# tyiannak/pyAudioAnalysis

Hardware: NVIDIA H100
Metric: audio frames/sec short-term feature_extraction @16kHz 50/25ms (higher is better)
Workload: dtype f32

## Files before the change

pyaudioanalysis_b200/csrc/b200aa.cu:

```cuda
#include <cuda_runtime.h>
#include <nvtx3/nvToolsExt.h>

#include <algorithm>
#include <atomic>
#include <cmath>
#include <cstdio>
#include <cstring>
#include <map>
#include <memory>
#include <mutex>
#include <string>
#include <vector>

#include "../../include/b200aa.h"
#include "beat.cuh"
#include "common.cuh"
#include "generic_kernel.cuh"
#include "fast_kernel.cuh"
#include "pair_kernel.cuh"
#include "pcm.cuh"
#include "solo_kernel.cuh"
#include "tables.inl"

using namespace b200aa;

static thread_local std::string g_cuda_err;
static std::atomic<int64_t> g_launches{0};

static int cuda_fail(cudaError_t e, const char *what)
{
    g_cuda_err = std::string(what) + ": " + cudaGetErrorString(e);
    return B200AA_ERR_CUDA;
}
#define CK(call)                                                     \
    do {                                                             \
        cudaError_t e_ = (call);                                     \
        if (e_ != cudaSuccess) return cuda_fail(e_, #call);          \
    } while (0)
#define CK_LAUNCH(name)                                              \
    do {                                                             \
        g_launches.fetch_add(1, std::memory_order_relaxed);          \
        cudaError_t e_ = cudaGetLastError();                         \
        if (e_ != cudaSuccess) return cuda_fail(e_, name);           \
    } while (0)

struct NvtxRange {
    explicit NvtxRange(const char *name) { nvtxRangePushA(name); }
    ~NvtxRange() { nvtxRangePop(); }
};

extern "C" int b200aa_abi_version(void) { return B200AA_ABI_VERSION; }
extern "C" int64_t b200aa_launch_count(void) { return g_launches.load(); }
extern "C" const char *b200aa_last_cuda_error(void) { return g_cuda_err.c_str(); }

extern "C" const char *b200aa_status_string(int s)
{
    switch (s) {
    case B200AA_OK: return "ok";
    case B200AA_ERR_INVALID: return "invalid argument";
    case B200AA_ERR_TOO_SHORT: return "need at least one array to concatenate";
    case B200AA_ERR_CHROMA: return "chroma: semitone index >= num_fft (window too short for this sampling rate)";
    case B200AA_ERR_MEL_RANGE: return "mel filterbank: filter edge beyond num_fft";
    case B200AA_ERR_CUDA: return "CUDA error";
    case B200AA_ERR_UNSUPPORTED: return "window too large for the on-chip transform";
    case B200AA_ERR_NO_DEVICE: return "no sm_90 CUDA device";
    default: return "unknown status";
    }
}

extern "C" int b200aa_device_ok(void)
{
    int dev = 0;
    if (cudaGetDevice(&dev) != cudaSuccess) { cudaGetLastError(); return B200AA_ERR_NO_DEVICE; }
    cudaDeviceProp pr;
    if (cudaGetDeviceProperties(&pr, dev) != cudaSuccess) { cudaGetLastError(); return B200AA_ERR_NO_DEVICE; }
    return (pr.major == 9 && pr.minor == 0) ? B200AA_OK : B200AA_ERR_NO_DEVICE;
}

extern "C" int b200aa_host_table(int fs, int window, int which, double *h_out)
{
    if (!h_out || window < 2 || fs <= 0) return B200AA_ERR_INVALID;
    const int K = window / 2;
    std::vector<double> t;
    int rc = B200AA_OK;
    if (which == 0) rc = b200aa_host::build_mel(fs, K, t);
    else if (which == 1) rc = b200aa_host::build_chroma(fs, K, t);
    else if (which == 2) b200aa_host::build_dct(t);
    else return B200AA_ERR_INVALID;
    if (rc != B200AA_OK) return rc;
    std::memcpy(h_out, t.data(), t.size() * sizeof(double));
    return B200AA_OK;
}

extern "C" int64_t b200aa_num_frames(int64_t n, int w, int s)
{
    return (w < 1 || s < 1) ? 0 : b200aa_host::num_frames(n, w, s);
}
extern "C" int64_t b200aa_spectrogram_rows(int64_t n, int w, int s)
{
    return (w < 1 || s < 1) ? 0 : rows::spectrogram(n, w, s).R;
}
extern "C" int64_t b200aa_chromagram_rows(int64_t n, int w, int s)
{
    return (w < 1 || s < 1) ? 0 : rows::chromagram(n, w, s).R;
}
__host__ __device__ inline int64_t frames_of(int64_t n, int w, int s) { return n < w ? 0 : (n - w) / s + 1; }
__host__ __device__ inline int64_t windows_of(int64_t n_frames, int stepr)
{
    return (stepr < 1 || n_frames <= 0) ? 0 : (n_frames + stepr - 1) / stepr;
}

extern "C" int64_t b200aa_mid_windows(int64_t n_frames, int stepr) { return windows_of(n_frames, stepr); }

struct Transform {
    int n = 0, Nc = 0, packed = 0;
    std::vector<int> radix;
    float2 *d_tw = nullptr, *d_tw_post = nullptr;
    ~Transform()
    {
        if (d_tw) cudaFree(d_tw);
        if (d_tw_post) cudaFree(d_tw_post);
    }
};

struct b200aa_plan {
    int fs = 0, window = 0, step = 0, K = 0;
    int device = 0, sm_count = 0;
    int force_generic = 0;
    int fast_kind = 0;
    int tables_status = B200AA_OK;
    BlobLayout bl{};
    int *d_blob = nullptr;
    std::vector<int> h_blob;
    std::mutex mu;
    std::map<int, std::unique_ptr<Transform>> transforms;
    std::mutex host_mu;
    void *ws[4] = {nullptr, nullptr, nullptr, nullptr};
    size_t ws_cap[4] = {0, 0, 0, 0};
    FastTables fast{};
    PairTables pair{};
    SoloTables solo{};
    int prefer = -1;
    static constexpr unsigned kSlots = 64;
    static constexpr size_t kSlotBytes = 64 * 1024;
    unsigned char *d_counters = nullptr;
    cudaEvent_t slot_event[kSlots] = {};
    bool slot_used[kSlots] = {};
    unsigned next_slot = 0;
    std::mutex slot_mu;
    static constexpr int kPipe = 3;
    cudaStream_t pipe_stream[kPipe] = {nullptr, nullptr, nullptr};
    void *pipe_ws[kPipe][3] = {};
    size_t pipe_cap[kPipe][3] = {};
    ~b200aa_plan()
    {
        if (d_blob) cudaFree(d_blob);
        for (void *w : ws) if (w) cudaFree(w);
        for (int k = 0; k < kPipe; ++k) {
            if (pipe_stream[k]) cudaStreamDestroy(pipe_stream[k]);
            for (void *w : pipe_ws[k]) if (w) cudaFree(w);
        }
        fast.release();
        pair.release();
        solo.release();
        if (d_counters) cudaFree(d_counters);
        for (cudaEvent_t e : slot_event) if (e) cudaEventDestroy(e);
    }
};

static int make_transform(int n, std::unique_ptr<Transform> &out)
{
    std::unique_ptr<Transform> t(new Transform);
    t->n = n;
    t->packed = (n % 2 == 0) ? 1 : 0;
    t->Nc = t->packed ? n / 2 : n;
    t->radix = b200aa_host::radix_list(t->Nc);
    if (t->Nc == 1) t->radix.clear();
    if ((int)t->radix.size() > kMaxRadix) return B200AA_ERR_UNSUPPORTED;
    std::vector<float2> tw(t->Nc), tp(t->Nc);
    for (int j = 0; j < t->Nc; ++j) {
        const double a = -2.0 * b200aa_host::kPi * double(j) / double(t->Nc);
        tw[j] = make_float2(float(std::cos(a)), float(std::sin(a)));
        const double b = -2.0 * b200aa_host::kPi * double(j) / double(n);
        tp[j] = make_float2(float(std::cos(b)), float(std::sin(b)));
    }
    CK(cudaMalloc(&t->d_tw, sizeof(float2) * t->Nc));
    CK(cudaMalloc(&t->d_tw_post, sizeof(float2) * t->Nc));
    CK(cudaMemcpy(t->d_tw, tw.data(), sizeof(float2) * t->Nc, cudaMemcpyHostToDevice));
    CK(cudaMemcpy(t->d_tw_post, tp.data(), sizeof(float2) * t->Nc, cudaMemcpyHostToDevice));
    out = std::move(t);
    return B200AA_OK;
}

static int get_transform(b200aa_plan *pl, int n, Transform **out)
{
    std::lock_guard<std::mutex> g(pl->mu);
    auto it = pl->transforms.find(n);
    if (it == pl->transforms.end()) {
        std::unique_ptr<Transform> t;
        int rc = make_transform(n, t);
        if (rc != B200AA_OK) return rc;
        it = pl->transforms.emplace(n, std::move(t)).first;
    }
    *out = it->second.get();
    return B200AA_OK;
}

extern "C" int b200aa_plan_create(b200aa_plan **out, int fs, int window, int step)
{
    if (!out || fs <= 0 || window < 2 || step < 1) return B200AA_ERR_INVALID;
    int rc = b200aa_device_ok();
    if (rc != B200AA_OK) return rc;
    std::unique_ptr<b200aa_plan> pl(new b200aa_plan);
    pl->fs = fs; pl->window = window; pl->step = step; pl->K = window / 2;
    CK(cudaGetDevice(&pl->device));
    CK(cudaDeviceGetAttribute(&pl->sm_count, cudaDevAttrMultiProcessorCount, pl->device));
    pl->tables_status = b200aa_host::build_blob(fs, pl->K, pl->h_blob, pl->bl);
    CK(cudaMalloc(&pl->d_blob, sizeof(int) * pl->h_blob.size()));
    CK(cudaMemcpy(pl->d_blob, pl->h_blob.data(), sizeof(int) * pl->h_blob.size(), cudaMemcpyHostToDevice));
    Transform *t = nullptr;
    rc = get_transform(pl.get(), window, &t);
    if (rc != B200AA_OK) return rc;
    rc = fast_plan_init(fs, window, step, pl->h_blob, pl->bl, &pl->fast, &pl->fast_kind);
    if (rc != B200AA_OK) return rc;
    int sl_ = 0, sr_ = 0;
    if ((pair_r_for_window(window) || solo_shape_for_window(window, &sl_, &sr_)) && pl->tables_status == B200AA_OK) {
        std::vector<double> mel, chr, dct;
        b200aa_host::build_mel(fs, pl->K, mel);
        b200aa_host::build_chroma(fs, pl->K, chr);
        b200aa_host::build_dct(dct);
        std::vector<int> pblob;
        PairBlobLayout pbl{};
        build_pair_blob(mel, chr, dct, pl->K, pblob, pbl);
        rc = pair_plan_init(window, pblob, pbl, &pl->pair);
        if (rc != B200AA_OK) return cuda_fail(cudaGetLastError(), "pair_plan_init");
        rc = solo_plan_init(window, pblob, pbl, &pl->solo);
        if (rc != B200AA_OK) return cuda_fail(cudaGetLastError(), "solo_plan_init");
    }
    CK(cudaMalloc(&pl->d_counters, b200aa_plan::kSlots * b200aa_plan::kSlotBytes));
    *out = pl.release();
    return B200AA_OK;
}

extern "C" void b200aa_plan_destroy(b200aa_plan *plan) { delete plan; }
static int slot_acquire(b200aa_plan *pl, cudaStream_t st, unsigned *slot, unsigned int **ctr)
{
    std::lock_guard<std::mutex> g(pl->slot_mu);
    const unsigned s = pl->next_slot++ % b200aa_plan::kSlots;
    if (!pl->slot_event[s]) CK(cudaEventCreateWithFlags(&pl->slot_event[s], cudaEventDisableTiming));
    if (pl->slot_used[s]) CK(cudaStreamWaitEvent(st, pl->slot_event[s], 0));
    *slot = s;
    *ctr = reinterpret_cast<unsigned int *>(pl->d_counters + size_t(s) * b200aa_plan::kSlotBytes);
    return B200AA_OK;
}
static int slot_done(b200aa_plan *pl, cudaStream_t st, unsigned slot)
{
    std::lock_guard<std::mutex> g(pl->slot_mu);
    CK(cudaEventRecord(pl->slot_event[slot], st));
    pl->slot_used[slot] = true;
    return B200AA_OK;
}

static bool use_pair(const b200aa_plan *pl) { return pl->pair.R && !pl->force_generic && (pl->prefer < 0 || pl->prefer == 2); }
static bool use_solo(const b200aa_plan *pl) { return pl->solo.L && !pl->force_generic && (pl->prefer < 0 || pl->prefer == 3); }
static bool use_fast(const b200aa_plan *pl) { return pl->fast_kind && !pl->force_generic && (pl->prefer < 0 || pl->prefer == 1); }
extern "C" int b200aa_plan_kernel_kind(const b200aa_plan *plan)
{
    if (!plan) return 0;
    return use_pair(plan) ? 2 : (use_solo(plan) ? 3 : (use_fast(plan) ? 1 : 0));
}
extern "C" int b200aa_plan_prefer_kernel(b200aa_plan *plan, int kind)
{
    if (!plan || kind < -1 || kind > 3) return B200AA_ERR_INVALID;
    plan->prefer = kind;
    return B200AA_OK;
}
static float *g_pair_dump = nullptr;
extern "C" int b200aa_debug_set_dump(float *d_rows)
{
    g_pair_dump = d_rows;
    return B200AA_OK;
}
extern "C" int b200aa_plan_force_generic(b200aa_plan *plan, int on)
{
    if (!plan) return 0;
    int prev = plan->force_generic;
    plan->force_generic = on ? 1 : 0;
    return prev;
}

extern "C" int b200aa_plan_trim(b200aa_plan *plan)
{
    if (!plan) return B200AA_ERR_INVALID;
    std::lock_guard<std::mutex> g(plan->host_mu);
    for (int i = 0; i < 4; ++i) {
        if (plan->ws[i]) cudaFree(plan->ws[i]);
        plan->ws[i] = nullptr; plan->ws_cap[i] = 0;
    }
    for (int k = 0; k < b200aa_plan::kPipe; ++k)
        for (int j = 0; j < 3; ++j) {
            if (plan->pipe_ws[k][j]) cudaFree(plan->pipe_ws[k][j]);
            plan->pipe_ws[k][j] = nullptr; plan->pipe_cap[k][j] = 0;
        }
    return B200AA_OK;
}

static int plan_device_check(const b200aa_plan *pl)
{
    int dev = -1;
    CK(cudaGetDevice(&dev));
    return dev == pl->device ? B200AA_OK : B200AA_ERR_INVALID;
}

__device__ __forceinline__ int float_key(float f)
{
    int b = __float_as_int(f);
    return b >= 0 ? b : b ^ 0x7fffffff;
}
__device__ __forceinline__ float key_float(int k) { return __int_as_float(k >= 0 ? k : k ^ 0x7fffffff); }

__global__ void stats_init_kernel(b200aa_clip_norm *nm, int64_t n)
{
    int64_t i = blockIdx.x * int64_t(blockDim.x) + threadIdx.x;
    if (i >= n) return;
    unsigned long long *acc = reinterpret_cast<unsigned long long *>(&nm[i].rsv[1]);
    *acc = 0ull;
    reinterpret_cast<int *>(&nm[i].lo)[0] = 0x7fffffff;
    reinterpret_cast<int *>(&nm[i].hi)[0] = int(0x80000000u);
}

template <int DTYPE>
__global__ void __launch_bounds__(256) stats_accum_kernel(const void *sig, int64_t n_samples, int64_t clip_stride,
                                                           const int64_t *len, b200aa_clip_norm *nm, int chunks)
{
    const int64_t b = blockIdx.y;
    const int64_t L = len ? len[b] : n_samples;
    const int64_t per = (L + chunks - 1) / chunks;
    const int64_t s0 = blockIdx.x * per, s1 = min(L, s0 + per);
    long long isum = 0;
    double dsum = 0.0;
    int kmin = 0x7fffffff, kmax = int(0x80000000u);
    if (DTYPE == B200AA_DTYPE_I16) {
        const short *x = reinterpret_cast<const short *>(sig) + b * clip_stride;
        int mn = 32767, mx = -32768;
        int64_t i = s0 + threadIdx.x;
        const bool al = ((reinterpret_cast<uintptr_t>(x + s0) & 15) == 0);
        if (al) {
            const int4 *v = reinterpret_cast<const int4 *>(x + s0);
            const int64_t nv = (s1 - s0) / 8;
            int64_t j = threadIdx.x;
            for (; j + 3 * int64_t(blockDim.x) < nv; j += 4 * int64_t(blockDim.x)) {
                int4 q[4];
#pragma unroll
                for (int t = 0; t < 4; ++t) q[t] = __ldg(v + j + t * int64_t(blockDim.x));
                int acc = 0;
#pragma unroll
                for (int t = 0; t < 4; ++t) {
                    const int w4[4] = {q[t].x, q[t].y, q[t].z, q[t].w};
#pragma unroll
                    for (int u = 0; u < 4; ++u) {
                        const int a0 = (short)(w4[u] & 0xffff), a1 = w4[u] >> 16;
                        acc += a0 + a1;
                        mn = min(mn, min(a0, a1));
                        mx = max(mx, max(a0, a1));
                    }
                }
                isum += acc;
            }
            for (; j < nv; j += blockDim.x) {
                int acc = 0;
                const int4 q = __ldg(v + j);
                const int w4[4] = {q.x, q.y, q.z, q.w};
#pragma unroll
                for (int u = 0; u < 4; ++u) {
                    const int a0 = (short)(w4[u] & 0xffff), a1 = w4[u] >> 16;
                    acc += a0 + a1;
                    mn = min(mn, min(a0, a1));
                    mx = max(mx, max(a0, a1));
                }
                isum += acc;
            }
            i = s0 + nv * 8 + threadIdx.x;
        }
        for (; i < s1; i += blockDim.x) {
            const int a0 = x[i];
            isum += a0;
            mn = min(mn, a0);
            mx = max(mx, a0);
        }
        kmin = mn; kmax = mx;
    } else {
        const float *x = reinterpret_cast<const float *>(sig) + b * clip_stride;
        for (int64_t i = s0 + threadIdx.x; i < s1; i += blockDim.x) {
            const float v = x[i];
            dsum += double(v);
            const int k = float_key(v);
            kmin = min(kmin, k);
            kmax = max(kmax, k);
        }
    }
    __shared__ long long s_i[8];
    __shared__ double s_d[8];
    __shared__ int s_mn[8], s_mx[8];
    const int lane = threadIdx.x & 31, warp = threadIdx.x >> 5;
#pragma unroll
    for (int o = 16; o > 0; o >>= 1) {
        isum += __shfl_xor_sync(0xffffffffu, isum, o);
        dsum += __shfl_xor_sync(0xffffffffu, dsum, o);
        kmin = min(kmin, __shfl_xor_sync(0xffffffffu, kmin, o));
        kmax = max(kmax, __shfl_xor_sync(0xffffffffu, kmax, o));
    }
    if (lane == 0) { s_i[warp] = isum; s_d[warp] = dsum; s_mn[warp] = kmin; s_mx[warp] = kmax; }
    __syncthreads();
    if (threadIdx.x == 0 && s1 > s0) {
        for (int w = 1; w < 8; ++w) { isum += s_i[w]; dsum += s_d[w]; kmin = min(kmin, s_mn[w]); kmax = max(kmax, s_mx[w]); }
        if (DTYPE == B200AA_DTYPE_I16)
            atomicAdd(reinterpret_cast<unsigned long long *>(&nm[b].rsv[1]), (unsigned long long)isum);
        else
            atomicAdd(reinterpret_cast<double *>(&nm[b].rsv[1]), dsum);
        atomicMin(reinterpret_cast<int *>(&nm[b].lo), kmin);
        atomicMax(reinterpret_cast<int *>(&nm[b].hi), kmax);
    }
}

template <int DTYPE>
__global__ void stats_finish_kernel(b200aa_clip_norm *nm, int64_t n, int64_t n_samples, const int64_t *len)
{
    int64_t i = blockIdx.x * int64_t(blockDim.x) + threadIdx.x;
    if (i >= n) return;
    const int64_t L = len ? len[i] : n_samples;
    b200aa_clip_norm r = nm[i];
    double mean, mn, mx;
    if (DTYPE == B200AA_DTYPE_I16) {
        const long long s = *reinterpret_cast<const long long *>(&nm[i].rsv[1]);
        mean = L > 0 ? double(s) / double(L) : 0.0;
        mn = double(*reinterpret_cast<const int *>(&r.lo));
        mx = double(*reinterpret_cast<const int *>(&r.hi));
    } else {
        const double s = *reinterpret_cast<const double *>(&nm[i].rsv[1]);
        mean = L > 0 ? s / double(L) : 0.0;
        mn = double(key_float(*reinterpret_cast<const int *>(&r.lo)));
        mx = double(key_float(*reinterpret_cast<const int *>(&r.hi)));
    }
    if (L <= 0) { mn = mx = 0.0; }
    const double maxdev = fmax(mx - mean, mean - mn);
    const double a = 1.0 / (maxdev + 32768.0 * 1e-10);
    double m, lo, hi;
    if (DTYPE == B200AA_DTYPE_I16) {
        m = nearbyint(mean);
        lo = floor(mean);
        hi = ceil(mean);
    } else {
        const float mf = float(mean);
        m = double(mf);
        if (double(mf) > mean) { hi = mf; lo = nextafterf(mf, -INFINITY); }
        else if (double(mf) < mean) { lo = mf; hi = nextafterf(mf, INFINITY); }
        else { lo = hi = mf; }
    }
    b200aa_clip_norm o;
    o.a = float(a);
    o.bp = float(a * (m - mean));
    o.m = float(m);
    o.lo = float(lo - m);
    o.hi = float(hi - m);
    o.rsv[0] = o.rsv[1] = o.rsv[2] = 0.f;
    nm[i] = o;
}

extern "C" int b200aa_clip_stats(const void *d_sig, int dtype, int64_t n_clips, int64_t n_samples,
                                 int64_t clip_stride, const int64_t *d_len, b200aa_clip_norm *d_norm, void *stream)
{
    NvtxRange nvtx_("b200aa_clip_stats");
    if (!d_sig || !d_norm || n_clips < 0 || n_samples < 0 || (dtype != 0 && dtype != 1)) return B200AA_ERR_INVALID;
    if (n_clips == 0) return B200AA_OK;
    cudaStream_t st = static_cast<cudaStream_t>(stream);
    int dev = 0, sms = 0;
    CK(cudaGetDevice(&dev));
    CK(cudaDeviceGetAttribute(&sms, cudaDevAttrMultiProcessorCount, dev));
    const int tb = 256;
    stats_init_kernel<<<(unsigned)((n_clips + tb - 1) / tb), tb, 0, st>>>(d_norm, n_clips);
    CK_LAUNCH("stats_init_kernel");
    int64_t want = (int64_t(sms) * 8 + n_clips - 1) / n_clips;
    const int64_t bytes = n_samples * (dtype == 0 ? 2 : 4);
    int64_t cap = (bytes + 32767) / 32768;
    int chunks = (int)std::max<int64_t>(1, std::min<int64_t>(want, cap));
    for (int64_t b0 = 0; b0 < n_clips; b0 += 32768) {
        const int64_t nb = std::min<int64_t>(32768, n_clips - b0);
        dim3 grid(chunks, (unsigned)nb);
        const size_t es = dtype == 0 ? 2 : 4;
        const void *sig = reinterpret_cast<const char *>(d_sig) + size_t(b0) * clip_stride * es;
        const int64_t *ln = d_len ? d_len + b0 : nullptr;
        if (dtype == 0) stats_accum_kernel<0><<<grid, 256, 0, st>>>(sig, n_samples, clip_stride, ln, d_norm + b0, chunks);
        else stats_accum_kernel<1><<<grid, 256, 0, st>>>(sig, n_samples, clip_stride, ln, d_norm + b0, chunks);
        CK_LAUNCH("stats_accum_kernel");
    }
    if (dtype == 0) stats_finish_kernel<0><<<(unsigned)((n_clips + tb - 1) / tb), tb, 0, st>>>(d_norm, n_clips, n_samples, d_len);
    else stats_finish_kernel<1><<<(unsigned)((n_clips + tb - 1) / tb), tb, 0, st>>>(d_norm, n_clips, n_samples, d_len);
    CK_LAUNCH("stats_finish_kernel");
    return B200AA_OK;
}

template <bool RAGGED>
__global__ void __launch_bounds__(256) mid_pool_kernel(const float *st, int64_t n_clips, int F, int64_t T,
                                                        int64_t t_stride, const int64_t *frames, int ratio, int stepr,
                                                        int64_t M, float *mid)
{
    const int lane = threadIdx.x & 31;
    const int64_t wid = (blockIdx.x * int64_t(blockDim.x) + threadIdx.x) >> 5;
    const int64_t total = n_clips * F * M;
    if (wid >= total) return;
    const int64_t j = wid % M, bf = wid / M;
    const int64_t b = bf / F;
    const int f = int(bf - b * F);
    if (RAGGED) {
        T = min(max(frames[b], int64_t(0)), t_stride);
        if (j >= windows_of(T, stepr)) return;
    }
    const int64_t c0 = j * stepr;
    int64_t c1 = min(T, c0 + ratio);
    if (c1 < 0) c1 = max(c1 + T, int64_t(0));
    const float *row = st + (size_t(b) * F + f) * t_stride;
    const int n = int(max(c1 - c0, int64_t(0)));
    double s = 0.0;
    for (int64_t c = c0 + lane; c < c1; c += 32) s += double(row[c]);
#pragma unroll
    for (int o = 16; o > 0; o >>= 1) s += __shfl_xor_sync(0xffffffffu, s, o);
    const double mean = s / double(n);
    double v = 0.0;
    for (int64_t c = c0 + lane; c < c1; c += 32) { const double d = double(row[c]) - mean; v += d * d; }
#pragma unroll
    for (int o = 16; o > 0; o >>= 1) v += __shfl_xor_sync(0xffffffffu, v, o);
    if (lane == 0) {
        float mu = float(mean), sd = float(sqrt(v / double(n)));
        if (isnan(mu)) mu = 0.f;
        if (isnan(sd)) sd = 0.f;
        if (isinf(mu)) mu = mu > 0 ? 3.4028234664e38f : -3.4028234664e38f;
        if (isinf(sd)) sd = 3.4028234664e38f;
        mid[(size_t(b) * 2 * F + f) * M + j] = mu;
        mid[(size_t(b) * 2 * F + F + f) * M + j] = sd;
    }
}

static int mid_pool_launch(const float *d_st, int64_t n_clips, int n_feats, int64_t T, int64_t t_stride, const int64_t *d_frames,
                           int ratio, int step_ratio, float *d_mid, void *stream)
{
    const int64_t M = windows_of(T, step_ratio);
    const int64_t warps = n_clips * n_feats * M;
    if (warps == 0) return B200AA_OK;
    const int64_t blocks = (warps * 32 + 255) / 256;
    auto kernel = d_frames ? mid_pool_kernel<true> : mid_pool_kernel<false>;
    kernel<<<(unsigned)blocks, 256, 0, static_cast<cudaStream_t>(stream)>>>(d_st, n_clips, n_feats, T, t_stride, d_frames,
                                                                             ratio, step_ratio, M, d_mid);
    CK_LAUNCH("mid_pool_kernel");
    return B200AA_OK;
}

extern "C" int b200aa_mid_pool(const float *d_st, int64_t n_clips, int n_feats, int64_t n_frames, int64_t t_stride,
                               int ratio, int step_ratio, float *d_mid, void *stream)
{
    NvtxRange nvtx_("b200aa_mid_pool");
    if (!d_st || !d_mid || n_clips < 0 || n_feats < 1 || n_frames < 1 || step_ratio < 1 || t_stride < n_frames)
        return B200AA_ERR_INVALID;
    return mid_pool_launch(d_st, n_clips, n_feats, n_frames, t_stride, nullptr, ratio, step_ratio, d_mid, stream);
}

extern "C" int b200aa_mid_pool_ragged(const float *d_st, int64_t n_clips, int n_feats, int64_t t_stride,
                                      const int64_t *d_frames, int ratio, int step_ratio, float *d_mid, void *stream)
{
    NvtxRange nvtx_("b200aa_mid_pool_ragged");
    if (!d_st || !d_frames || !d_mid || n_clips < 0 || n_feats < 1 || step_ratio < 1 || t_stride < 0)
        return B200AA_ERR_INVALID;
    return mid_pool_launch(d_st, n_clips, n_feats, t_stride, t_stride, d_frames, ratio, step_ratio, d_mid, stream);
}

__global__ void __launch_bounds__(256) long_term_mean_kernel(const float *mid, int64_t rows_total, int n_rows, int64_t M,
                                                             const int64_t *windows, float *out)
{
    const int lane = threadIdx.x & 31;
    const int64_t wid = (blockIdx.x * int64_t(blockDim.x) + threadIdx.x) >> 5;
    if (wid >= rows_total) return;
    const int64_t Mb = windows ? min(max(windows[wid / n_rows], int64_t(0)), M) : M;
    const float *row = mid + size_t(wid) * M;
    double s = 0.0;
    for (int64_t c = lane; c < Mb; c += 32) s += double(row[c]);
#pragma unroll
    for (int o = 16; o > 0; o >>= 1) s += __shfl_xor_sync(0xffffffffu, s, o);
    if (lane == 0) out[wid] = float(s / double(Mb));
}

static int long_term_mean_launch(const float *d_mid, int64_t n_clips, int n_rows, int64_t m_stride, const int64_t *d_windows,
                                 float *d_out, void *stream)
{
    const int64_t rows = n_clips * n_rows;
    if (rows == 0) return B200AA_OK;
    const int64_t blocks = (rows * 32 + 255) / 256;
    long_term_mean_kernel<<<(unsigned)blocks, 256, 0, static_cast<cudaStream_t>(stream)>>>(d_mid, rows, n_rows, m_stride,
                                                                                             d_windows, d_out);
    CK_LAUNCH("long_term_mean_kernel");
    return B200AA_OK;
}

extern "C" int b200aa_long_term_mean(const float *d_mid, int64_t n_clips, int n_rows, int64_t n_windows, float *d_out, void *stream)
{
    if (!d_mid || !d_out || n_clips < 0 || n_rows < 1 || n_windows < 1) return B200AA_ERR_INVALID;
    return long_term_mean_launch(d_mid, n_clips, n_rows, n_windows, nullptr, d_out, stream);
}

extern "C" int b200aa_long_term_mean_ragged(const float *d_mid, int64_t n_clips, int n_rows, int64_t m_stride,
                                            const int64_t *d_windows, float *d_out, void *stream)
{
    if (!d_mid || !d_windows || !d_out || n_clips < 0 || n_rows < 1 || m_stride < 0) return B200AA_ERR_INVALID;
    return long_term_mean_launch(d_mid, n_clips, n_rows, m_stride, d_windows, d_out, stream);
}

__global__ void __launch_bounds__(256) frame_counts_kernel(const int64_t *len, int64_t n_clips, int w, int s, int stepr,
                                                           int64_t *frames, int64_t *windows)
{
    const int64_t b = blockIdx.x * int64_t(blockDim.x) + threadIdx.x;
    if (b >= n_clips) return;
    const int64_t T = frames_of(len[b], w, s);
    frames[b] = T;
    if (windows) windows[b] = windows_of(T, stepr);
}

extern "C" int b200aa_frame_counts(const int64_t *d_len, int64_t n_clips, int window, int step, int step_ratio,
                                   int64_t *d_frames, int64_t *d_windows, void *stream)
{
    if (!d_len || !d_frames || n_clips < 0 || window < 1 || step < 1 || (d_windows && step_ratio < 1))
        return B200AA_ERR_INVALID;
    if (n_clips == 0) return B200AA_OK;
    const int64_t blocks = (n_clips + 255) / 256;
    frame_counts_kernel<<<(unsigned)blocks, 256, 0, static_cast<cudaStream_t>(stream)>>>(d_len, n_clips, window, step,
                                                                                           step_ratio, d_frames, d_windows);
    CK_LAUNCH("frame_counts_kernel");
    return B200AA_OK;
}

__global__ void __launch_bounds__(256) row_counts_kernel(const int64_t *len, int64_t n_clips, int w, int s, int which, int64_t *out)
{
    const int64_t b = blockIdx.x * int64_t(blockDim.x) + threadIdx.x;
    if (b >= n_clips) return;
    const rows::Rows r = which ? rows::chromagram(len[b], w, s) : rows::spectrogram(len[b], w, s);
    out[b] = r.refused ? 0 : r.R;
}

extern "C" int b200aa_row_counts(const int64_t *d_len, int64_t n_clips, int window, int step, int which, int64_t *d_rows,
                                 void *stream)
{
    if (!d_len || !d_rows || n_clips < 0 || window < 1 || step < 1 || (which != 0 && which != 1)) return B200AA_ERR_INVALID;
    if (n_clips == 0) return B200AA_OK;
    const int64_t blocks = (n_clips + 255) / 256;
    row_counts_kernel<<<(unsigned)blocks, 256, 0, static_cast<cudaStream_t>(stream)>>>(d_len, n_clips, window, step, which, d_rows);
// ... 713 lines not shown
```

pyaudioanalysis_b200/csrc/pair_kernel.cuh:

```cuda
#pragma once
#include "common.cuh"
#include "dft_codelets.cuh"
#include <algorithm>
#include <cstring>
#include <utility>
#include "fast_kernel.cuh"
#include "sched.cuh"

namespace b200aa {

#ifndef B200AA_PAIR_MAXWARPS
#define B200AA_PAIR_MAXWARPS 24
#endif
constexpr int kPairMaxWarps = B200AA_PAIR_MAXWARPS;
#ifndef B200AA_PAIR_MINBLOCKS
#define B200AA_PAIR_MINBLOCKS 1
#endif
constexpr int kPairMinBlocks = B200AA_PAIR_MINBLOCKS;
#ifndef B200AA_SOLO_MAXWARPS
#define B200AA_SOLO_MAXWARPS 24
#endif
#ifndef B200AA_SOLO_MINBLOCKS
#define B200AA_SOLO_MINBLOCKS 1
#endif
// ... 241 lines not shown
}

template <int P, int NV, int D, int NA>
__device__ __forceinline__ void mr_halve(float (&v)[NA], int lane)
{
    if constexpr (P > 1) {
        constexpr int H = P / 2;
        const bool up = lane & D;
#pragma unroll
        for (int i = 0; i < H; ++i) {
            if (i < NV) {
                if (i + H < NV) {
                    const float keep = up ? v[i + H] : v[i], send = up ? v[i] : v[i + H];
                    v[i] = keep + __shfl_xor_sync(0xffffffffu, send, D);
                } else {
                    v[i] += __shfl_xor_sync(0xffffffffu, v[i], D);
                }
            }
        }
        mr_halve<H, (NV < H ? NV : H), D / 2, NA>(v, lane);
    } else {
#pragma unroll
        for (int d = D; d >= 1; d >>= 1) v[0] += __shfl_xor_sync(0xffffffffu, v[0], d);
    }
}
template <int NV>
struct MultiReduce {
    static constexpr int P0 = NV > 16 ? 32 : (NV > 8 ? 16 : 8);
    static constexpr int SH = NV > 16 ? 0 : (NV > 8 ? 1 : 2);
    __device__ static __forceinline__ void run(float (&v)[NV], int lane) { mr_halve<P0, NV, 16, NV>(v, lane); }
};

template <int R, bool FULL>
struct TdShape {
    using S = PairShape<R>;
    static constexpr int NREST = (S::N % 10) ? 1 : 0;
    static constexpr int NE = FULL ? 10 + NREST : 5;
    static constexpr int EB = FULL ? 0 : 5;
    static constexpr int NFIRST = FULL ? 0 : S::N / 2;
    static constexpr int ROW0 = NFIRST / 32, LANE0 = NFIRST % 32;
    static constexpr int ZROW0 = (!FULL && LANE0 == 0) ? ROW0 - 1 : ROW0;
    static_assert(FULL || S::kShareable, "half-frame sharing needs whole blocks per half");
};

template <int R, bool FULL, bool TWO>
__device__ __forceinline__ void td_pair(const float2 (&u)[R], float cm, const b200aa_clip_norm &nm, int lane,
                                        float2 *e2 , int &flips_a, int &link_a, int &flips_b, int &link_b,
                                        int (*half_flips)[4] = nullptr)
{
    using S = PairShape<R>;
    using Td = TdShape<R, FULL>;
    constexpr int N = S::N, Lt = S::Lt, NH = N / 2, HROW0 = NH / 32, HLANE0 = NH % 32;
    unsigned pPa = 0u, pQa = 0u, pPb = 0u, pQb = 0u;
    int fa = 0, la = 0, fb = 0, lb = 0;
    int hfa = 0, hla = 0, hfb = 0, hlb = 0;
    const float2 ncm = make_float2(-cm, -cm), a2 = make_float2(nm.a, nm.a), bp2 = make_float2(nm.bp, nm.bp);
#pragma unroll
    for (int r = Td::ZROW0; r < R; ++r) {
        const float2 d = f2add(u[r], ncm);
        const unsigned Pa = __ballot_sync(0xffffffffu, d.x > nm.lo), Pb = __ballot_sync(0xffffffffu, d.y > nm.lo);
        unsigned Qa = 0u, Qb = 0u;
        if (TWO) { Qa = __ballot_sync(0xffffffffu, d.x < nm.hi); Qb = __ballot_sync(0xffffffffu, d.y < nm.hi); }
        if (FULL && r == 0) { pPa = (Pa & 1u) << 31; pQa = (Qa & 1u) << 31; pPb = (Pb & 1u) << 31; pQb = (Qb & 1u) << 31; }
        if (r >= Td::ROW0) {
            const int n0 = 32 * r;
            const int nstart = FULL ? 1 : Td::NFIRST;
            const unsigned valid = n0 >= nstart ? 0xffffffffu : (n0 + 32 <= nstart ? 0u : (0xffffffffu << (nstart - n0)));
            const unsigned cPa = (Pa ^ __funnelshift_l(pPa, Pa, 1)) & valid, cPb = (Pb ^ __funnelshift_l(pPb, Pb, 1)) & valid;
            fa += __popc(cPa); fb += __popc(cPb);
            if (!FULL && r == Td::ROW0) { la += int((cPa >> Td::LANE0) & 1u); lb += int((cPb >> Td::LANE0) & 1u); }
            unsigned cQa = 0u, cQb = 0u;
            if (TWO) {
                cQa = (Qa ^ __funnelshift_l(pQa, Qa, 1)) & valid; cQb = (Qb ^ __funnelshift_l(pQb, Qb, 1)) & valid;
                fa += __popc(cQa); fb += __popc(cQb);
                if (!FULL && r == Td::ROW0) { la += int((cQa >> Td::LANE0) & 1u); lb += int((cQb >> Td::LANE0) & 1u); }
            }
            if (FULL && r >= HROW0) {
                const unsigned hv = n0 >= NH ? 0xffffffffu : (0xffffffffu << (NH - n0));
                hfa += __popc(cPa & hv) + __popc(cQa & hv); hfb += __popc(cPb & hv) + __popc(cQb & hv);
                if (r == HROW0) {
                    hla += int((cPa >> HLANE0) & 1u) + int((cQa >> HLANE0) & 1u);
                    hlb += int((cPb >> HLANE0) & 1u) + int((cQb >> HLANE0) & 1u);
                }
            }
            const float2 y = f2fma(a2, d, bp2);
            const bool live = !(r == Td::ROW0 && Td::LANE0 > 0) || lane >= Td::LANE0;
            const int b0 = (n0 / Lt) < 10 ? (n0 / Lt) : 10;
            const int end = b0 < 10 ? (b0 + 1) * Lt : N;
            const int thr = end - n0;
            const int i0 = b0 - Td::EB, i1 = (b0 + 1 < 10 ? b0 + 1 : 10) - Td::EB;
            if (thr >= 32) {
                if (i0 >= 0 && i0 < Td::NE) { if (live) e2[i0] = f2fma(y, y, e2[i0]); }
            } else {
                const bool first = lane < thr;
                if (i0 >= 0 && i0 < Td::NE) { if (live && first) e2[i0] = f2fma(y, y, e2[i0]); }
                if (i1 >= 0 && i1 < Td::NE) { if (live && !first) e2[i1] = f2fma(y, y, e2[i1]); }
            }
        }
        pPa = Pa; pQa = Qa; pPb = Pb; pQb = Qb;
    }
    flips_a = TWO ? fa : 2 * fa; link_a = TWO ? la : 2 * la;
    flips_b = TWO ? fb : 2 * fb; link_b = TWO ? lb : 2 * lb;
    if (FULL && half_flips) {
        const int m = TWO ? 1 : 2;
        (*half_flips)[0] = m * hfa; (*half_flips)[1] = m * hla; (*half_flips)[2] = m * hfb; (*half_flips)[3] = m * hlb;
    }
}

__device__ __forceinline__ void frame_scale(float E, float inv_a2n, float &s, float &inv_s)
{
    const float t = E * inv_a2n;
    const int ex = (__float_as_int(t) >> 23) & 0xff;
    int k = (127 - ex) >> 1;
    k = k < -30 ? -30 : (k > 40 ? 40 : k);
    s = __int_as_float((127 + k) << 23);
    inv_s = __int_as_float((127 - k) << 23);
}

struct FeatTables {
    const float *dct;
    const int *mrec;
    const float4 *mw;
    const int2 *chr;
    int LQ, CT;
};

template <int K>
__device__ __forceinline__ void rows_to_features(const float *Xa, const float *Xb, const float *Xprev, bool fresh, float carried,
                                                 const int *dlane, float *parts, float *msraw, float *mslog, float *mfold, float *chr,
                                                 float *fva, float *fvb, const FeatTables &ft, int lane)
{
    const int half = lane >> 4, l16 = lane & 15;
    const unsigned FULLM = 0xffffffffu;
    {
        const float *X = half ? Xb : Xa;
        const float *Xp = half ? Xa : Xprev;
        pair_spectral<K>(X, Xp, carried, fresh, dlane + l16 * 4, parts + half * 32, half ? fvb : fva, l16, half);
    }
    {
        const float *X = half ? Xb : Xa;
        float acc = 0.f;
#pragma unroll 4
        for (int q = 0; q < ft.LQ; ++q) {
            const int rec = ft.mrec[q * 16 + l16];
            const float4 w = ft.mw[q * 16 + l16];
            const float *xp = X + (rec & 0xffff);
            acc = fmaf(xp[0], w.x, acc);
            acc = fmaf(xp[1], w.y, acc);
            acc = fmaf(xp[2], w.z, acc);
            acc = fmaf(xp[3], w.w, acc);
            if (rec & (1 << 24)) { msraw[half * B200AA_N_MEL + ((rec >> 16) & 0xff)] = acc; acc = 0.f; }
        }
        float ch = 0.f;
        for (int t = 0; t < ft.CT; ++t) {
            const int2 e = ft.chr[t * 16 + l16];
            const float v = X[e.x];
            ch = fmaf(v * v, __int_as_float(e.y), ch);
        }
        if (l16 < 12) chr[half * 12 + l16] = ch;
    }
    __syncwarp();
#pragma unroll
    for (int t = lane; t < 2 * B200AA_N_MEL; t += 32) mslog[t] = 0.30102999566398120f * flog2(msraw[t] + B200AA_EPS);
    __syncwarp();
#pragma unroll
    for (int t = lane; t < 2 * B200AA_N_MEL; t += 32) {
        const int f = t >= B200AA_N_MEL ? 1 : 0, r = t - f * B200AA_N_MEL;
        const int kind = r >= 20 ? 1 : 0, n = r - 20 * kind;
        const float *m = mslog + f * B200AA_N_MEL;
        const float a = m[n], bq = m[39 - n], kap = m[0];
        mfold[t] = kind ? a - bq : (a - kap) + (bq - kap);
    }
    __syncwarp();
    {
        const int c = l16 < B200AA_N_MFCC ? l16 : 0;
        const float *src = mfold + half * B200AA_N_MEL + 20 * (c & 1);
        const float *row = ft.dct + c * 41;
        float acc = 0.f;
#pragma unroll
        for (int n = 0; n < 20; ++n) acc = fmaf(row[n], src[n], acc);
        if (c == 0) acc = fmaf(6.324555320336759f, mslog[half * B200AA_N_MEL], acc);
        if (l16 < B200AA_N_MFCC) (half ? fvb : fva)[8 + c] = acc;
    }
    chroma_finalize_h(chr + half * 12, half ? fvb : fva, l16, true);
    __syncwarp();
    (void)FULLM;
}

__device__ __forceinline__ void tile_store(const float *fv, int tile_n, int tile_t0, float *out_clip, int64_t t_stride, int n_out, int lane)
{
    const int c = lane & 7, f0 = lane >> 3;
    if (c < tile_n) {
        float *out_f = out_clip + f0 * t_stride + (tile_t0 + c);
        const int64_t step4 = 4 * t_stride, delta = B200AA_N_BASE * t_stride;
        const float *cur_row = fv + (1 + c) * kFvStride, *prv_row = fv + c * kFvStride;
        const bool first = tile_t0 + c == 0;
#pragma unroll
        for (int i = 0; i < 9; ++i) {
            const int f = f0 + 4 * i;
            if (f < B200AA_N_BASE) {
                const float v = cur_row[f];
                out_f[0] = v;
                if (n_out > B200AA_N_BASE) out_f[delta] = first ? 0.f : v - prv_row[f];
            }
            out_f += step4;
        }
    }
}

__device__ __forceinline__ void tile_flush(float *fv, int &tile_n, int &tile_t0, float *out_clip, int64_t t_stride, int n_out, int lane)
{
    if (tile_n > 0) {
        tile_store(fv, tile_n, tile_t0, out_clip, t_stride, n_out, lane);
        __syncwarp();
        fv[lane] = fv[tile_n * kFvStride + lane];
        if (lane < 4) fv[32 + lane] = fv[tile_n * kFvStride + 32 + lane];
        tile_t0 += tile_n;
        tile_n = 0;
        __syncwarp();
    }
}

template <int R, bool SHARED>
__global__ void __launch_bounds__(32 * pair_warps<R>(), kPairMinBlocks) st_pair_kernel(const PairParams pp)
{
    using S = PairShape<R>;
    constexpr int N = S::N, K = S::K, Kp = S::Kp, C = S::C, JK = S::JK, LS = S::LS;
    static_assert(!SHARED || S::kShareable, "shared halves need N % 160 == 0");
    extern __shared__ __align__(16) unsigned char smem_raw[];
    PairCtaMem<R> &cm_ = *reinterpret_cast<PairCtaMem<R> *>(smem_raw);
    int *const blob_s = reinterpret_cast<int *>(smem_raw + sizeof(PairCtaMem<R>));
    const StParams &p = pp.st;
    const int tid = threadIdx.x, lane = tid & 31, warp = tid >> 5;
    constexpr int NTHR = 32 * pair_warps<R>();
#pragma unroll 1
    for (int i = tid; i < pp.pbl.words; i += NTHR) blob_s[i] = pp.pblob[i];
#pragma unroll 1
    for (int i = tid; i < R * 32; i += NTHR) cm_.tw[i] = pp.tw[i];
    if (tid < 16) *reinterpret_cast<int4 *>(cm_.dlane + tid * 4) = pair_lane_init<K>(tid);
    __syncthreads();
    const float *const t_dct = reinterpret_cast<const float *>(blob_s + pp.pbl.dct);
    const int *const t_mrec = blob_s + pp.pbl.mel_rec;
    const float4 *const t_mw = reinterpret_cast<const float4 *>(blob_s + pp.pbl.mel_w);
    const int2 *const t_chr = reinterpret_cast<const int2 *>(blob_s + pp.pbl.chr);
    const FeatTables ftab{t_dct, t_mrec, t_mw, t_chr, pp.pbl.lq, pp.pbl.ct};
    PairWarpMem<R> &wm = cm_.w[warp];
    float *const rowa = reinterpret_cast<float *>(wm.tz);
    float *const t_re = reinterpret_cast<float *>(wm.tz), *const t_im = t_re + R * LS;
    float *const msraw = rowa + S::MS0, *const mslog = msraw + 2 * B200AA_N_MEL, *const mfold = mslog + 2 * B200AA_N_MEL;
    const int step = p.step;
    const int half = lane >> 4, l16 = lane & 15;
    const unsigned FULLM = 0xffffffffu;

    const unsigned wglob = blockIdx.x * unsigned(pair_warps<R>()) + unsigned(warp);
    if (lane == 0) sched_begin(pp.sched, wglob);
    __syncwarp();
    const unsigned per_clip = pp.sched.per_clip;
    const bool is16 = p.dtype == B200AA_DTYPE_I16;
    const float M0 = is16 ? 8421376.f : 0.f;
    unsigned inc = pp.sched.chunk;
    unsigned g0 = 0, g1 = 0;
    unsigned run_b = 0xffffffffu, run_q = 0xffffffffu;
    int q = 0, q0 = 0, q1 = 0;
    int tile_n = 0, tile_t0 = 0;
    int zprev = 0;
    bool fresh = false;
    const char *clip = nullptr;
    int T = 0, NP = 0;
    b200aa_clip_norm nm{};
    float cmv = 0.f;
    bool two_sided = false;
    for (;;) {
        bool flush = false;
        if (q < q1) {
            const bool store = q >= q0;
            const int ta = 2 * q;
            const bool bvalid = ta + 1 < T;
            float2 uab[R];
            {
                unsigned int wa[R], wb[R];
                const int oa = ta * step + lane, ob = (bvalid ? ta + 1 : ta) * step + lane;
                if (is16) {
                    const unsigned short *const s16 = reinterpret_cast<const unsigned short *>(clip);
#pragma unroll
                    for (int r = 0; r < R; ++r) { wa[r] = __ldg(s16 + oa + 32 * r); wb[r] = __ldg(s16 + ob + 32 * r); }
                } else {
                    const unsigned int *const s32 = reinterpret_cast<const unsigned int *>(clip);
#pragma unroll
                    for (int r = 0; r < R; ++r) { wa[r] = __ldg(s32 + oa + 32 * r); wb[r] = __ldg(s32 + ob + 32 * r); }
                }
                if (is16) {
#pragma unroll
                    for (int r = 0; r < R; ++r)
                        uab[r] = make_float2(__int_as_float(0x4B000000 | (int(wa[r]) ^ 0x8000)), __int_as_float(0x4B000000 | (int(wb[r]) ^ 0x8000)));
                } else {
#pragma unroll
                    for (int r = 0; r < R; ++r) uab[r] = make_float2(__int_as_float(wa[r]), __int_as_float(wb[r]));
                }
            }
            const float u0a = __shfl_sync(FULLM, uab[0].x, 0), u0b = __shfl_sync(FULLM, uab[0].y, 0);
            const int ra = store ? 1 + tile_n : 8, rb = store ? 2 + tile_n : 0;
            float *const fva = wm.fv + ra * kFvStride, *const fvb = wm.fv + rb * kFvStride;

            const bool a_full = !SHARED || fresh;
            int fl_a, fl_b;
            {
// ... 426 lines not shown
```

Measured before the change: 366.1 million.

## Fuse clip stats init/accum/finish into one cluster or last-block-reduce kernel

Replaces the three-kernel clip-statistics path (init, atomic accumulate, finish) with a single kernel. Up to eight chunk blocks per clip reduce their partials through thread-block-cluster distributed shared memory, and larger chunk counts use a global scratch buffer with a last-arriving-block reduction. This removes two launches and the global atomics, at the cost of a stream-ordered malloc/free and cluster launch constraints. It also adds an unroll pragma to the chroma accumulation loop in the pair kernel.

```diff
diff --git a/pyaudioanalysis_b200/csrc/b200aa.cu b/pyaudioanalysis_b200/csrc/b200aa.cu
--- a/pyaudioanalysis_b200/csrc/b200aa.cu
+++ b/pyaudioanalysis_b200/csrc/b200aa.cu
@@ -1,3 +1,4 @@
+#include <cooperative_groups.h>
 #include <cuda_runtime.h>
 #include <nvtx3/nvToolsExt.h>
 
@@ -23,6 +24,7 @@
 #include "tables.inl"
 
 using namespace b200aa;
+namespace cg = cooperative_groups;
 
 static thread_local std::string g_cuda_err;
 static std::atomic<int64_t> g_launches{0};
@@ -319,24 +321,26 @@
 }
 __device__ __forceinline__ float key_float(int k) { return __int_as_float(k >= 0 ? k : k ^ 0x7fffffff); }
 
-__global__ void stats_init_kernel(b200aa_clip_norm *nm, int64_t n)
-{
-    int64_t i = blockIdx.x * int64_t(blockDim.x) + threadIdx.x;
-    if (i >= n) return;
-    unsigned long long *acc = reinterpret_cast<unsigned long long *>(&nm[i].rsv[1]);
-    *acc = 0ull;
-    reinterpret_cast<int *>(&nm[i].lo)[0] = 0x7fffffff;
-    reinterpret_cast<int *>(&nm[i].hi)[0] = int(0x80000000u);
+struct StatsPart {
+    long long isum;
+    double dsum;
+    int kmin, kmax;
+    int any;
+};
+constexpr int kStatsCluster = 8;
+constexpr int kStatsThreads = 256;
+
+__device__ __forceinline__ void stats_add(StatsPart &t, long long isum, double dsum, int kmin, int kmax, int any)
+{
+    if (!any) return;
+    t.isum += isum; t.dsum += dsum;
+    t.kmin = min(t.kmin, kmin); t.kmax = max(t.kmax, kmax);
+    t.any = 1;
 }
 
 template <int DTYPE>
-__global__ void __launch_bounds__(256) stats_accum_kernel(const void *sig, int64_t n_samples, int64_t clip_stride,
-                                                           const int64_t *len, b200aa_clip_norm *nm, int chunks)
-{
-    const int64_t b = blockIdx.y;
-    const int64_t L = len ? len[b] : n_samples;
-    const int64_t per = (L + chunks - 1) / chunks;
-    const int64_t s0 = blockIdx.x * per, s1 = min(L, s0 + per);
+__device__ __forceinline__ StatsPart stats_chunk(const void *sig, int64_t b, int64_t clip_stride, int64_t s0, int64_t s1)
+{
     long long isum = 0;
     double dsum = 0.0;
     int kmin = 0x7fffffff, kmax = int(0x80000000u);
@@ -399,9 +403,9 @@
             kmax = max(kmax, k);
         }
     }
-    __shared__ long long s_i[8];
-    __shared__ double s_d[8];
-    __shared__ int s_mn[8], s_mx[8];
+    __shared__ long long s_i[kStatsThreads / 32];
+    __shared__ double s_d[kStatsThreads / 32];
+    __shared__ int s_mn[kStatsThreads / 32], s_mx[kStatsThreads / 32];
     const int lane = threadIdx.x & 31, warp = threadIdx.x >> 5;
 #pragma unroll
     for (int o = 16; o > 0; o >>= 1) {
@@ -412,35 +416,24 @@
     }
     if (lane == 0) { s_i[warp] = isum; s_d[warp] = dsum; s_mn[warp] = kmin; s_mx[warp] = kmax; }
     __syncthreads();
-    if (threadIdx.x == 0 && s1 > s0) {
-        for (int w = 1; w < 8; ++w) { isum += s_i[w]; dsum += s_d[w]; kmin = min(kmin, s_mn[w]); kmax = max(kmax, s_mx[w]); }
-        if (DTYPE == B200AA_DTYPE_I16)
-            atomicAdd(reinterpret_cast<unsigned long long *>(&nm[b].rsv[1]), (unsigned long long)isum);
-        else
-            atomicAdd(reinterpret_cast<double *>(&nm[b].rsv[1]), dsum);
-        atomicMin(reinterpret_cast<int *>(&nm[b].lo), kmin);
-        atomicMax(reinterpret_cast<int *>(&nm[b].hi), kmax);
-    }
+    StatsPart r{isum, dsum, kmin, kmax, s1 > s0 ? 1 : 0};
+    if (threadIdx.x == 0)
+        for (int w = 1; w < kStatsThreads / 32; ++w) { r.isum += s_i[w]; r.dsum += s_d[w]; r.kmin = min(r.kmin, s_mn[w]); r.kmax = max(r.kmax, s_mx[w]); }
+    return r;
 }
 
 template <int DTYPE>
-__global__ void stats_finish_kernel(b200aa_clip_norm *nm, int64_t n, int64_t n_samples, const int64_t *len)
-{
-    int64_t i = blockIdx.x * int64_t(blockDim.x) + threadIdx.x;
-    if (i >= n) return;
-    const int64_t L = len ? len[i] : n_samples;
-    b200aa_clip_norm r = nm[i];
+__device__ b200aa_clip_norm stats_record(const StatsPart &t, int64_t L)
+{
     double mean, mn, mx;
     if (DTYPE == B200AA_DTYPE_I16) {
-        const long long s = *reinterpret_cast<const long long *>(&nm[i].rsv[1]);
-        mean = L > 0 ? double(s) / double(L) : 0.0;
-        mn = double(*reinterpret_cast<const int *>(&r.lo));
-        mx = double(*reinterpret_cast<const int *>(&r.hi));
+        mean = L > 0 ? double(t.isum) / double(L) : 0.0;
+        mn = double(t.kmin);
+        mx = double(t.kmax);
     } else {
-        const double s = *reinterpret_cast<const double *>(&nm[i].rsv[1]);
-        mean = L > 0 ? s / double(L) : 0.0;
-        mn = double(key_float(*reinterpret_cast<const int *>(&r.lo)));
-        mx = double(key_float(*reinterpret_cast<const int *>(&r.hi)));
+        mean = L > 0 ? t.dsum / double(L) : 0.0;
+        mn = double(key_float(t.kmin));
+        mx = double(key_float(t.kmax));
     }
     if (L <= 0) { mn = mx = 0.0; }
     const double maxdev = fmax(mx - mean, mean - mn);
@@ -464,7 +457,45 @@
     o.lo = float(lo - m);
     o.hi = float(hi - m);
     o.rsv[0] = o.rsv[1] = o.rsv[2] = 0.f;
-    nm[i] = o;
+    return o;
+}
+
+template <int DTYPE, bool SPLIT>
+__global__ void __launch_bounds__(kStatsThreads) clip_stats_kernel(const void *sig, int64_t n_samples, int64_t clip_stride,
+                                                                   const int64_t *len, b200aa_clip_norm *nm,
+                                                                   StatsPart *parts, unsigned int *arrived)
+{
+    const int64_t b = blockIdx.y;
+    const int chunks = gridDim.x;
+    const int64_t L = len ? len[b] : n_samples;
+    const int64_t per = (L + chunks - 1) / chunks;
+    const int64_t s0 = blockIdx.x * per, s1 = min(L, s0 + per);
+    const StatsPart mine = stats_chunk<DTYPE>(sig, b, clip_stride, s0, s1);
+    StatsPart t{0, 0.0, 0x7fffffff, int(0x80000000u), 0};
+    if constexpr (!SPLIT) {
+        __shared__ StatsPart s_part;
+        cg::cluster_group cl = cg::this_cluster();
+        if (threadIdx.x == 0) s_part = mine;
+        cl.sync();
+        if (cl.block_rank() == 0 && threadIdx.x == 0) {
+            for (int r = 0; r < chunks; ++r) {
+                const StatsPart &q = *cl.map_shared_rank(&s_part, r);
+                stats_add(t, q.isum, q.dsum, q.kmin, q.kmax, q.any);
+            }
+            nm[b] = stats_record<DTYPE>(t, L);
+        }
+        cl.sync();
+    } else {
+        if (threadIdx.x != 0) return;
+        StatsPart *const cp = parts + b * chunks;
+        cp[blockIdx.x] = mine;
+        __threadfence();
+        if (atomicAdd(&arrived[b], 1u) != unsigned(chunks - 1)) return;
+        __threadfence();
+        for (int r = 0; r < chunks; ++r)
+            stats_add(t, __ldcg(&cp[r].isum), __ldcg(&cp[r].dsum), __ldcg(&cp[r].kmin), __ldcg(&cp[r].kmax), __ldcg(&cp[r].any));
+        nm[b] = stats_record<DTYPE>(t, L);
+    }
 }
 
 extern "C" int b200aa_clip_stats(const void *d_sig, int dtype, int64_t n_clips, int64_t n_samples,
@@ -477,27 +508,55 @@
     int dev = 0, sms = 0;
     CK(cudaGetDevice(&dev));
     CK(cudaDeviceGetAttribute(&sms, cudaDevAttrMultiProcessorCount, dev));
-    const int tb = 256;
-    stats_init_kernel<<<(unsigned)((n_clips + tb - 1) / tb), tb, 0, st>>>(d_norm, n_clips);
-    CK_LAUNCH("stats_init_kernel");
     int64_t want = (int64_t(sms) * 8 + n_clips - 1) / n_clips;
     const int64_t bytes = n_samples * (dtype == 0 ? 2 : 4);
     int64_t cap = (bytes + 32767) / 32768;
-    int chunks = (int)std::max<int64_t>(1, std::min<int64_t>(want, cap));
+    const int chunks = (int)std::max<int64_t>(1, std::min<int64_t>(want, cap));
+    const bool split = chunks > kStatsCluster;
+    StatsPart *parts = nullptr;
+    unsigned int *arrived = nullptr;
+    if (split) {
+        const size_t pb = sizeof(StatsPart) * size_t(chunks) * size_t(n_clips);
+        void *scratch = nullptr;
+        CK(cudaMallocAsync(&scratch, pb + sizeof(unsigned int) * size_t(n_clips), st));
+        parts = static_cast<StatsPart *>(scratch);
+        arrived = reinterpret_cast<unsigned int *>(static_cast<char *>(scratch) + pb);
+        const cudaError_t e = cudaMemsetAsync(arrived, 0, sizeof(unsigned int) * size_t(n_clips), st);
+        if (e != cudaSuccess) { cudaFreeAsync(scratch, st); return cuda_fail(e, "cudaMemsetAsync"); }
+    }
+    const size_t es = dtype == 0 ? 2 : 4;
+    int rc = B200AA_OK;
     for (int64_t b0 = 0; b0 < n_clips; b0 += 32768) {
         const int64_t nb = std::min<int64_t>(32768, n_clips - b0);
-        dim3 grid(chunks, (unsigned)nb);
-        const size_t es = dtype == 0 ? 2 : 4;
+        cudaLaunchConfig_t cfg = {};
+        cfg.gridDim = dim3(chunks, (unsigned)nb);
+        cfg.blockDim = dim3(kStatsThreads);
+        cfg.stream = st;
+        cudaLaunchAttribute at[1];
+        at[0].id = cudaLaunchAttributeClusterDimension;
+        at[0].val.clusterDim.x = chunks;
+        at[0].val.clusterDim.y = 1;
+        at[0].val.clusterDim.z = 1;
+        cfg.attrs = at;
+        cfg.numAttrs = split ? 0 : 1;
         const void *sig = reinterpret_cast<const char *>(d_sig) + size_t(b0) * clip_stride * es;
         const int64_t *ln = d_len ? d_len + b0 : nullptr;
-        if (dtype == 0) stats_accum_kernel<0><<<grid, 256, 0, st>>>(sig, n_samples, clip_stride, ln, d_norm + b0, chunks);
-        else stats_accum_kernel<1><<<grid, 256, 0, st>>>(sig, n_samples, clip_stride, ln, d_norm + b0, chunks);
-        CK_LAUNCH("stats_accum_kernel");
-    }
-    if (dtype == 0) stats_finish_kernel<0><<<(unsigned)((n_clips + tb - 1) / tb), tb, 0, st>>>(d_norm, n_clips, n_samples, d_len);
-    else stats_finish_kernel<1><<<(unsigned)((n_clips + tb - 1) / tb), tb, 0, st>>>(d_norm, n_clips, n_samples, d_len);
-    CK_LAUNCH("stats_finish_kernel");
-    return B200AA_OK;
+        StatsPart *pp = split ? parts + b0 * chunks : nullptr;
+        unsigned int *ap = split ? arrived + b0 : nullptr;
+        cudaError_t e;
+        if (dtype == 0) e = split ? cudaLaunchKernelEx(&cfg, clip_stats_kernel<0, true>, sig, n_samples, clip_stride, ln, d_norm + b0, pp, ap)
+                                  : cudaLaunchKernelEx(&cfg, clip_stats_kernel<0, false>, sig, n_samples, clip_stride, ln, d_norm + b0, pp, ap);
+        else e = split ? cudaLaunchKernelEx(&cfg, clip_stats_kernel<1, true>, sig, n_samples, clip_stride, ln, d_norm + b0, pp, ap)
+                       : cudaLaunchKernelEx(&cfg, clip_stats_kernel<1, false>, sig, n_samples, clip_stride, ln, d_norm + b0, pp, ap);
+        g_launches.fetch_add(1, std::memory_order_relaxed);
+        if (e == cudaSuccess) e = cudaGetLastError();
+        if (e != cudaSuccess) { rc = cuda_fail(e, "clip_stats_kernel"); break; }
+    }
+    if (parts) {
+        const cudaError_t e = cudaFreeAsync(parts, st);
+        if (e != cudaSuccess && rc == B200AA_OK) rc = cuda_fail(e, "cudaFreeAsync");
+    }
+    return rc;
 }
 
 template <bool RAGGED>
diff --git a/pyaudioanalysis_b200/csrc/pair_kernel.cuh b/pyaudioanalysis_b200/csrc/pair_kernel.cuh
--- a/pyaudioanalysis_b200/csrc/pair_kernel.cuh
+++ b/pyaudioanalysis_b200/csrc/pair_kernel.cuh
@@ -417,6 +417,7 @@
             if (rec & (1 << 24)) { msraw[half * B200AA_N_MEL + ((rec >> 16) & 0xff)] = acc; acc = 0.f; }
         }
         float ch = 0.f;
+#pragma unroll 4
         for (int t = 0; t < ft.CT; ++t) {
             const int2 e = ft.chr[t * 16 + l16];
             const float v = X[e.x];
```

After: 367.4 million, median of 6. Within noise of the previous version (+0.4%).
